# player4771/YOLO-DBL

Measured on AMD Instinct MI355X. Metric: images/sec @640×640 bs=32 (1/2/4/8 GPU) + mAP@0.5 vs CPU ref, higher is better.
Workload: dtype fp16; 1 GPU; YOLO-DBL-n 640x640 bs=32/GPU fp16 forward+decode+NMS (conf .25, iou .7, max_det 300); model=yolov13n_DBL, global_batch=32, imgsz=640, nc=3, parallelism=dp1, streams_per_gpu=2

## Files before the change

### yolo-dbl_amd/csrc/bneck_kernel.hpp

```cpp
#pragma once
#include <algorithm>

#include "common.hpp"
#ifdef YDBL_BNECK_SPARSE
#include "decode_math.hpp"
#endif

namespace ydbl {

struct KSlot {
  int tap, chunk;
  bool live;
};

template <int CH>
__host__ __device__ constexpr KSlot kslot(int m, int g) {
  if constexpr (CH >= 4) {
    return KSlot{m / (CH / 4), (m % (CH / 4)) * 4 + g, true};
  } else if constexpr (CH == 2) {
    const int tap = 2 * m + (g >> 1);
    return KSlot{tap < 9 ? tap : 8, g & 1, tap < 9};
  } else {
    constexpr int taps[3][4] = {{0, 3, 1, 4}, {2, 5, 6, 6}, {7, 7, 8, 8}};
    constexpr bool live[3][4] = {{true, true, true, true}, {true, true, true, false}, {true, false, true, false}};
    return KSlot{taps[m][g], 0, live[m][g]};
  }
}
template <int CH>
constexpr int ksteps() {
  return CH >= 4 ? 9 * CH / 4 : (CH == 2 ? 5 : 3);
}
constexpr int rup16(int v) { return (v + 15) / 16 * 16; }

template <int C, int CMID, int TH, int CIN = C>
struct BneckCfg {
  static constexpr int CM = CMID, CH = CIN / 8, CHM = (CM + 7) / 8;
  static constexpr int NT1 = (CM + 15) / 16, NT2 = C / 16;
  static constexpr bool BD = CM == 8 && CH == 2;
  static constexpr int KS1 = BD ? 9 : ksteps<CH>(), KS2 = ksteps<CHM>();
  static constexpr int TW = 16;
  static constexpr int IP = TW + 4;
  static constexpr int IR = TH + 5;
  static constexpr int NPX = IR * IP;
  static constexpr int PIN = rup16(NPX);
  static constexpr int MR = TH + 2;
  static constexpr int MP = CHM == 1 ? 32 : IP;
  static constexpr int PMID = rup16(MR * MP);
  static constexpr int G1 = (MR * IP + 15) / 16;
  static constexpr int IN_BYTES = CH * PIN * 16, MID_BYTES = CHM * PMID * 16;
  static constexpr int LDS = IN_BYTES + MID_BYTES;
  static constexpr int W1F = NT1 * KS1 * 64, W2F = NT2 * KS2 * 64;
  static constexpr int64_t BYTES = (int64_t)(W1F + W2F) * 16 + (NT1 * 16 + C) * 4;
  static_assert(CH >= 2, "input needs >= 16 channels");
  static_assert((G1 * 16 - 1) + 2 * IP + 2 < NPX, "virtual grid tail must stay inside the window");
};

template <int C, int CMID, int CIN = C>
void bneck_pack(const float* w1, const float* b1, const float* w2, const float* b2, unsigned char* out) {
  using Cfg = BneckCfg<C, CMID, 16, CIN>;
  constexpr int CM = Cfg::CM;
  _Float16* f1 = reinterpret_cast<_Float16*>(out);
  _Float16* f2 = f1 + Cfg::W1F * 8;
  float* fb1 = reinterpret_cast<float*>(f2 + Cfg::W2F * 8);
  float* fb2 = fb1 + Cfg::NT1 * 16;
  if constexpr (Cfg::BD) {
    for (int m = 0; m < Cfg::KS1; ++m)
      for (int lane = 0; lane < 64; ++lane)
        for (int j = 0; j < 8; ++j) {
          const int g = lane >> 4, row = lane & 15;
          const int co = row % 8, ci = (g & 1) * 8 + j;
          f1[(m * 64 + lane) * 8 + j] = (_Float16)((row / 8) == (g >> 1) ? w1[(co * CIN + ci) * 9 + m] : 0.f);
        }
  } else
  for (int t = 0; t < Cfg::NT1; ++t)
    for (int m = 0; m < Cfg::KS1; ++m)
      for (int lane = 0; lane < 64; ++lane)
        for (int j = 0; j < 8; ++j) {
          const KSlot s = kslot<Cfg::CH>(m, lane >> 4);
          const int co = 16 * t + (lane & 15), ci = s.chunk * 8 + j;
          const bool ok = s.live && co < CM;
          f1[((t * Cfg::KS1 + m) * 64 + lane) * 8 + j] = (_Float16)(ok ? w1[(co * CIN + ci) * 9 + s.tap] : 0.f);
        }
  for (int t = 0; t < Cfg::NT2; ++t)
    for (int m = 0; m < Cfg::KS2; ++m)
      for (int lane = 0; lane < 64; ++lane)
        for (int j = 0; j < 8; ++j) {
          const KSlot s = kslot<Cfg::CHM>(m, lane >> 4);
          const int co = 16 * t + (lane & 15), ci = s.chunk * 8 + j;
          const bool ok = s.live && ci < CM;
          f2[((t * Cfg::KS2 + m) * 64 + lane) * 8 + j] = (_Float16)(ok ? w2[(co * CM + ci) * 9 + s.tap] : 0.f);
        }
  for (int i = 0; i < Cfg::NT1 * 16; ++i) fb1[i] = i < CM ? b1[i] : 0.f;
  for (int i = 0; i < C; ++i) fb2[i] = b2[i];
}

template <int CH, int PL, int P>
__device__ __forceinline__ int koff(int m, int g) {
  const KSlot s = kslot<CH>(m, CH >= 4 ? 0 : g);
  return (s.chunk * PL + (s.tap / 3) * P + s.tap % 3) * 16;
}
template <int CH, int PL>
__device__ __forceinline__ int kbase(int g) {
  return CH >= 4 ? g * PL * 16 : 0;
}

#if defined(YDBL_BNECK_STAMPS) && defined(YDBL_BNECK_SPARSE)
#undef YDBL_BNECK_STAMPS
#endif
#ifdef YDBL_BNECK_STAMPS
__device__ unsigned long long g_bn_stamps[8 * 16384];
#define BN_STAMP(k)                                                                                         \
  do {                                                                                                    \
    if (threadIdx.x == 0 && blockIdx.x < 16384) g_bn_stamps[blockIdx.x * 8 + (k)] = __builtin_amdgcn_s_memrealtime(); \
  } while (0)
#else
#define BN_STAMP(k) \
  do {              \
  } while (0)
#endif

#ifdef YDBL_BNECK_SPARSE
struct BoxSink {
  const unsigned char* mask;
  float* cbox;
  const int* cidx;
  const int* ccount;
  int cap, a0, nc, multi;
  float stride;
};
constexpr int BOX_PITCH = 72, BOX_HITS = 512;

#define YDBL_BNECK_KERNEL bneck_sparse_kernel
#define YDBL_BNECK_SINK_ARG , BoxSink sk
#else
#define YDBL_BNECK_KERNEL bneck_kernel
#define YDBL_BNECK_SINK_ARG
#endif

template <int C, int CMID, int TH, bool ADD, bool PW = false, int CIN = C>
__global__ __launch_bounds__(256, 2) void YDBL_BNECK_KERNEL(DView<const _Float16> x, DView<_Float16> y,
                                                            const unsigned char* __restrict__ params, int tiles_x,
                                                            int tiles_y, int ntiles YDBL_BNECK_SINK_ARG) {
  using Cfg = BneckCfg<C, CMID, TH, CIN>;
#ifdef YDBL_BNECK_SPARSE
  static_assert(PW, "the tile mask belongs to the Detect box launch");
#endif
  constexpr int CH = Cfg::CH, CHM = Cfg::CHM, CM = Cfg::CM;
  static_assert(CIN == C || !ADD, "the residual needs c_in == c");
  constexpr bool LATE_A2 = CIN > C;
  constexpr int IP = Cfg::IP, MP = Cfg::MP, PIN = Cfg::PIN, PMID = Cfg::PMID;
  constexpr int NT1 = Cfg::NT1, NT2 = Cfg::NT2, KS1 = Cfg::KS1, KS2 = Cfg::KS2;
  const h8* w1f = reinterpret_cast<const h8*>(params);
  const h8* w2f = w1f + Cfg::W1F;
  const float* b1 = reinterpret_cast<const float*>(w2f + Cfg::W2F);
  const float* b2 = b1 + NT1 * 16;
  __shared__ __align__(16) unsigned char smem[Cfg::LDS];
  unsigned char* s_in = smem;
  unsigned char* s_mid = smem + Cfg::IN_BYTES;

  const int tid = threadIdx.x, lane = tid & 63, wave = wave_id();
  const int g = lane >> 4, r16 = lane & 15;
  BN_STAMP(0);
#ifdef YDBL_BNECK_STAMPS
  if (tid == 0 && blockIdx.x < 16384) {
    unsigned hw, xcc;
    asm volatile("s_getreg_b32 %0, hwreg(HW_REG_HW_ID)" : "=s"(hw));
    asm volatile("s_getreg_b32 %0, hwreg(HW_REG_XCC_ID)" : "=s"(xcc));
    g_bn_stamps[blockIdx.x * 8 + 4] = hw;
    g_bn_stamps[blockIdx.x * 8 + 5] = xcc;
  }
#endif
  const int t = (ntiles & 7) ? (int)blockIdx.x : xcd_remap(blockIdx.x, ntiles);
  const int tx = t % tiles_x, ty = (t / tiles_x) % tiles_y;
  const int img = t / (tiles_x * tiles_y);
  const int oy0 = ty * TH, ox0 = tx * Cfg::TW;
#ifdef YDBL_BNECK_SPARSE
  if (sk.mask[t] == 0) return;
  __shared__ int s_nhit;
  if (tid == 0) s_nhit = 0;
  int ncand = 0, idx0 = -1;
  if (sk.ccount) {
    ncand = min(sk.ccount[img], sk.cap);
    idx0 = sk.cidx[(int64_t)img * sk.cap + min(tid, sk.cap - 1)];
  }
#endif

  static_assert(32 % CH == 0, "staging pattern assumes CH | 32");
  constexpr int PXU = 256 / CH;
  constexpr int IT = (Cfg::NPX + PXU - 1) / PXU;
  const int s_chunk = (tid >> 3) % CH, px0 = ((tid >> 3) / CH) * 8 + (tid & 7);
  h8 xr[IT];
#pragma unroll
  for (int u = 0; u < IT; ++u) {
    const int px = px0 + u * PXU;
    const int r = px / IP, c = px - r * IP;
    const int iy = oy0 - 2 + r, ix = ox0 - 2 + c;
    const bool ok = px < Cfg::NPX && iy >= 0 && iy < x.h && ix >= 0 && ix < x.w;
    const _Float16* src = ok ? x.at(img, iy, ix) + s_chunk * 8 : x.p;
    const h8 v = *reinterpret_cast<const h8*>(src);
    xr[u] = ok ? v : h8{0, 0, 0, 0, 0, 0, 0, 0};
  }
  const int t1 = wave % NT1, t2 = wave % NT2;
  h8 a1[KS1], a2[KS2];
#pragma unroll
  for (int m = 0; m < KS1; ++m) a1[m] = w1f[(t1 * KS1 + m) * 64 + lane];
  if constexpr (!LATE_A2) {
#pragma unroll
    for (int m = 0; m < KS2; ++m) a2[m] = w2f[(t2 * KS2 + m) * 64 + lane];
  }
  unsigned char* s_dst = s_in + (s_chunk * PIN + px0) * 16;
#pragma unroll
  for (int u = 0; u < IT; ++u)
    if (px0 + u * PXU < Cfg::NPX) *reinterpret_cast<h8*>(s_dst + u * PXU * 16) = xr[u];
  float bias1[4], bias2[4];
  const int c1 = Cfg::BD ? 4 * (g & 1) : 16 * t1 + 4 * g;
  const int c2 = 16 * t2 + 4 * g;
#pragma unroll
  for (int q = 0; q < 4; ++q) {
    bias1[q] = b1[c1 + q];
    bias2[q] = b2[c2 + q];
  }
  unsigned char* mid_w = s_mid + ((c1 >> 3) * PMID) * 16 + (c1 & 7) * 2;
  const unsigned char* in_b = s_in + kbase<CH, PIN>(g);
  const bool interior = oy0 >= 1 && ox0 >= 1 && oy0 + TH + 1 <= y.h && ox0 + Cfg::TW + 1 <= y.w;
  __syncthreads();
  BN_STAMP(1);

  auto epi1 = [&](const f32x4& acc, int vr, int vc, int rb) {
    if (vr >= Cfg::MR || c1 >= CM) return;
    bool inside = true;
    if (!interior) {
      const int my = oy0 - 1 + vr, mx = ox0 - 1 + vc;
      inside = my >= 0 && my < y.h && mx >= 0 && mx < y.w;
    }
    h4 o;
#pragma unroll
    for (int q = 0; q < 4; ++q) {
      const float sv = silu_fast(acc[q] + bias1[q]);
      o[q] = f16_rne(inside ? sv : 0.f);
    }
    *reinterpret_cast<h4*>(mid_w + (rb + vc) * 16) = o;
  };
  constexpr int WPT1 = 4 / NT1;
  constexpr int S0 = 2 * WPT1 * 16, H1 = WPT1 * 16;
  int r0, c0, rb0;
  {
    const int v = (wave / NT1) * 16 + r16;
    r0 = v / IP;
    c0 = v - r0 * IP;
    rb0 = r0 * MP;
  }
  for (int gi = wave / NT1; gi < Cfg::G1; gi += 2 * WPT1) {
    const int v0 = gi * 16 + r16;
    const bool two = gi + WPT1 < Cfg::G1;
    const int v1 = two ? v0 + 16 * WPT1 : v0;
    if constexpr (Cfg::BD) {
      const int set = g >> 1;
      const unsigned char* pb = s_in + ((g & 1) * PIN + (set ? v1 : v0)) * 16;
      f32x4 acc = f32x4{0.f, 0.f, 0.f, 0.f};
#pragma unroll
      for (int m = 0; m < KS1; ++m) {
        const h8 bf = *reinterpret_cast<const h8*>(pb + ((m / 3) * IP + m % 3) * 16);
        acc = __builtin_amdgcn_mfma_f32_16x16x32_f16(a1[m], bf, acc, 0, 0, 0);
      }
      const bool w1 = c0 + H1 % IP >= IP;
      const int dr = set ? H1 / IP + (w1 ? 1 : 0) : 0;
      epi1(acc, set && !two ? Cfg::MR : r0 + dr, set ? c0 + H1 % IP - (w1 ? IP : 0) : c0, rb0 + dr * MP);
    } else {
      f32x4 acc0 = f32x4{0.f, 0.f, 0.f, 0.f}, acc1 = acc0;
      const unsigned char* p0 = in_b + v0 * 16;
      const unsigned char* p1 = in_b + v1 * 16;
#pragma unroll
      for (int m = 0; m < KS1; ++m) {
        const int o = koff<CH, PIN, IP>(m, g);
        const h8 bf0 = *reinterpret_cast<const h8*>(p0 + o);
        const h8 bf1 = *reinterpret_cast<const h8*>(p1 + o);
        acc0 = __builtin_amdgcn_mfma_f32_16x16x32_f16(a1[m], bf0, acc0, 0, 0, 0);
        acc1 = __builtin_amdgcn_mfma_f32_16x16x32_f16(a1[m], bf1, acc1, 0, 0, 0);
      }
      epi1(acc0, r0, c0, rb0);
      if (two) {
        const bool w1 = c0 + H1 % IP >= IP;
        const int dr = H1 / IP + (w1 ? 1 : 0);
        epi1(acc1, r0 + dr, c0 + H1 % IP - (w1 ? IP : 0), rb0 + dr * MP);
      }
    }
    const bool w0 = c0 + S0 % IP >= IP;
    const int dr = S0 / IP + (w0 ? 1 : 0);
    c0 += S0 % IP - (w0 ? IP : 0);
    r0 += dr;
    rb0 += dr * MP;
  }

  const unsigned char* res_r = s_in + ((c2 >> 3) * PIN + 2 * IP + 2) * 16 + (c2 & 7) * 2;
  const unsigned char* mid_b = s_mid + kbase<CHM, PMID>(g);
  if constexpr (LATE_A2) {
#pragma unroll
    for (int m = 0; m < KS2; ++m) a2[m] = w2f[(t2 * KS2 + m) * 64 + lane];
  }
  __syncthreads();
  BN_STAMP(2);

  const int64_t lane_px = (int64_t)r16 * y.cs;
  auto epi2 = [&](const f32x4& acc, int j) {
    const int oy = oy0 + j, ox = ox0 + r16;
    if (oy >= y.h || ox >= y.w) return;
    float v[4];
#pragma unroll
    for (int q = 0; q < 4; ++q) v[q] = silu_fast(acc[q] + bias2[q]);
    if constexpr (ADD) {
      const h4 rv = *reinterpret_cast<const h4*>(res_r + (j * IP + r16) * 16);
#pragma unroll
      for (int q = 0; q < 4; ++q) v[q] = float(rv[q]) + v[q];
    }
    if constexpr (PW) {
      h4 o;
#pragma unroll
      for (int q = 0; q < 4; ++q) o[q] = f16_rne(v[q]);
      *reinterpret_cast<h4*>(s_in + ((c2 >> 3) * (TH * 16) + j * 16 + r16) * 16 + (c2 & 7) * 2) = o;
    } else {
      store_f<4>(y.at(img, oy, ox0) + lane_px + c2, v);
    }
  };
  constexpr int WPT2 = 4 / NT2;
  for (int j = wave / NT2; j < TH; j += 2 * WPT2) {
    const bool two = j + WPT2 < TH;
    const int j1 = two ? j + WPT2 : j;
    f32x4 acc0 = f32x4{0.f, 0.f, 0.f, 0.f}, acc1 = acc0;
    const unsigned char* p0 = mid_b + (j * MP + r16) * 16;
    const unsigned char* p1 = mid_b + (j1 * MP + r16) * 16;
#pragma unroll
    for (int m = 0; m < KS2; ++m) {
      const int o = koff<CHM, PMID, MP>(m, g);
      const h8 bf0 = *reinterpret_cast<const h8*>(p0 + o);
      const h8 bf1 = *reinterpret_cast<const h8*>(p1 + o);
      acc0 = __builtin_amdgcn_mfma_f32_16x16x32_f16(a2[m], bf0, acc0, 0, 0, 0);
      acc1 = __builtin_amdgcn_mfma_f32_16x16x32_f16(a2[m], bf1, acc1, 0, 0, 0);
    }
    epi2(acc0, j);
    if (two) epi2(acc1, j1);
  }
  BN_STAMP(3);

  if constexpr (PW) {
    static_assert(ADD == false && C % 32 == 0 && (C / 8) * TH * 16 * 16 <= Cfg::IN_BYTES, "pw stage layout");
    constexpr int NT3 = C / 16, KS3 = C / 32, WPT3 = 4 / NT3;
    const h8* w3f = reinterpret_cast<const h8*>(b2 + C);
    const float* b3 = reinterpret_cast<const float*>(w3f + NT3 * KS3 * 64);
    const int t3 = wave % NT3, c3 = 16 * t3 + 4 * g;
    h8 a3[KS3];
#pragma unroll
    for (int m = 0; m < KS3; ++m) a3[m] = w3f[(t3 * KS3 + m) * 64 + lane];
    float bias3[4];
#pragma unroll
    for (int q = 0; q < 4; ++q) bias3[q] = b3[c3 + q];
    __syncthreads();
#ifdef YDBL_BNECK_SPARSE
    _Float16* s_box = reinterpret_cast<_Float16*>(s_mid);
    int* s_hit = reinterpret_cast<int*>(s_mid + TH * 16 * BOX_PITCH * 2);
    static_assert(C == 64 && TH * 16 * BOX_PITCH * 2 + BOX_HITS * 4 <= Cfg::MID_BYTES, "sink layout");
#endif
    for (int j = wave / NT3; j < TH; j += WPT3) {
      f32x4 acc = f32x4{0.f, 0.f, 0.f, 0.f};
#pragma unroll
      for (int m = 0; m < KS3; ++m) {
        const h8 bf = *reinterpret_cast<const h8*>(s_in + ((m * 4 + g) * (TH * 16) + j * 16 + r16) * 16);
        acc = __builtin_amdgcn_mfma_f32_16x16x32_f16(a3[m], bf, acc, 0, 0, 0);
      }
      const int oy = oy0 + j, ox = ox0 + r16;
      if (oy < y.h && ox < y.w) {
        float v[4];
#pragma unroll
        for (int q = 0; q < 4; ++q) v[q] = acc[q] + bias3[q];
#ifdef YDBL_BNECK_SPARSE
        const h4 o = to_h4_rne(v);
        *reinterpret_cast<h4*>(y.at(img, oy, ox) + c3) = o;
        *reinterpret_cast<h4*>(s_box + (j * 16 + r16) * BOX_PITCH + c3) = o;
#else
        store_f<4>(y.at(img, oy, ox) + c3, v);
#endif
      }
    }
#ifdef YDBL_BNECK_SPARSE
    {
      if (sk.ccount == nullptr) return;
      const int hw = y.h * y.w;
      const int* ci = sk.cidx + (int64_t)img * sk.cap;
      for (int i = tid; i < ncand; i += 256) {
        const int idx = i == tid ? idx0 : ci[i];
        const int loc = (sk.multi ? idx / sk.nc : idx) - sk.a0;
        if (loc < 0 || loc >= hw) continue;
        const int gy = loc / y.w, gx = loc - gy * y.w;
        const int jy = gy - oy0, jx = gx - ox0;
        if (jy < 0 || jy >= TH || jx < 0 || jx >= 16) continue;
        const int h = atomicAdd(&s_nhit, 1);
        if (h < BOX_HITS) s_hit[h] = (i << 7) | (jy * 16 + jx);
      }
      __syncthreads();
      const int nh = min(s_nhit, BOX_HITS);
      const int s = tid & 3;
      for (int h0 = 0; h0 < nh; h0 += 64) {
        const int h = h0 + (tid >> 2);
        const bool live = h < nh;
        const int e = s_hit[live ? h : 0];
        const int px = e & 127;
        const float mine = dfl_side(s_box + px * BOX_PITCH + s * 16);
        const int q0 = lane - s;
        float dist[4];
#pragma unroll
        for (int k = 0; k < 4; ++k) dist[k] = __shfl(mine, q0 + k);
        const f32x4 box = xywh2xyxy(dist2xywh(ox0 + (px & 15), oy0 + (px >> 4), dist, sk.stride));
        if (live && s == 0) *reinterpret_cast<f32x4*>(sk.cbox + ((int64_t)img * sk.cap + (e >> 7)) * 4) = box;
      }
    }
#endif
  }
}

}
```

### yolo-dbl_amd/csrc/sparse_box.hip

```cpp
#define YDBL_DS_DEFER
#define YDBL_BNECK_SPARSE
#include "bneck_kernel.hpp"
#include "dsc_lean.hpp"
#include "dsconv_kernel.hpp"

namespace ydbl {

template <int TH, int CSEG, bool DBUF>
static void ds_defer_go(const ConvArgs<_Float16>& a, const float* dww, const float* dwb, int dw_act, hipStream_t s) {
  const int tiles_x = (int)cdiv(a.Wo, 8), tiles_y = (int)cdiv(a.Ho, TH);
  const int64_t ntiles = (int64_t)a.N * tiles_y * tiles_x;
  dsconv_defer_kernel<_Float16, 3, 1, 1, TH, 8, CSEG, 4, DBUF, true><<<(unsigned)ntiles, 256, 0, s>>>(
      a, dww, dwb, dw_act, tiles_x, tiles_y, 1);
}

bool ds_defer_tile(const ConvArgs<_Float16>& a, const float* dww, const float* dwb, int dw_act, int th, int cseg,
                   bool dbuf, hipStream_t s) {
  if (!a.sk_deferred() || a.Cout != 64) return false;
  if (th == 8 && cseg == 2 && !dbuf) return ds_defer_go<8, 2, false>(a, dww, dwb, dw_act, s), true;
  if (th == 16 && cseg == 4 && !dbuf) return ds_defer_go<16, 4, false>(a, dww, dwb, dw_act, s), true;
  if (th == 8 && cseg == 2 && dbuf) return ds_defer_go<8, 2, true>(a, dww, dwb, dw_act, s), true;
  return false;
}

__global__ __launch_bounds__(256, 1) void dsc_lean_defer_kernel(ConvArgs<_Float16> p, const float* __restrict__ dww,
                                                                 const float* __restrict__ dwb, int dw_act, int tiles_x,
                                                                 int tiles_y, int ntiles) {
  __shared__ __attribute__((aligned(16))) unsigned char smem[LeanLds<64, 64, 3, 1, 8, 8, 256, true>::BYTES];
  lean_tile<64, 64, 3, 1, 8, 8, 256, true, true>(p, dww, dwb, dw_act, xcd_remap(blockIdx.x, ntiles), tiles_x, tiles_y,
                                                 smem);
}

void lean_defer_tile(const ConvArgs<_Float16>& a, const float* dww, const float* dwb, int dw_act, hipStream_t s) {
  const int tiles_x = (int)cdiv(a.Wo, 8), tiles_y = (int)cdiv(a.Ho, 8);
  const int ntiles = a.N * tiles_y * tiles_x;
  dsc_lean_defer_kernel<<<(unsigned)ntiles, 256, 0, s>>>(a, dww, dwb, dw_act, tiles_x, tiles_y, ntiles);
}

__global__ void ds_zero_counts_masks_kernel(int* c, int n, unsigned char* m, int nm) {
  for (int i = threadIdx.x; i < n; i += blockDim.x) c[i] = 0;
  for (int i = threadIdx.x; i < nm; i += blockDim.x) m[i] = 0;
}

void ds_zero_counts_masks(int* counts, int n, unsigned char* masks, int nbytes, hipStream_t s) {
  ds_zero_counts_masks_kernel<<<1, 256, 0, s>>>(counts, n, masks, nbytes);
}

template <int CIN>
static int box_sparse_go(const ydbl_bottleneck_desc* d, hipStream_t s) {
  using Cfg = BneckCfg<64, 64, 8, CIN>;
  const int tiles_x = (int)cdiv(d->y.w, Cfg::TW), tiles_y = (int)cdiv(d->y.h, 8);
  const int64_t nt = (int64_t)tiles_x * tiles_y * d->y.n;
  if (nt > 0x7fffffff) return fail(YDBL_EINVAL, "bottleneck: grid too large");
  const BoxSink sk{d->tile_mask, d->cand_box, d->cand_idx, d->cand_count, d->cand_cap, d->anchor0, d->nc,
                   d->multi_label, d->level_stride};
  bneck_sparse_kernel<64, 64, 8, false, true, CIN><<<(unsigned)nt, 256, 0, s>>>(
      dview<const _Float16>(d->x), dview<_Float16>(d->y), reinterpret_cast<const unsigned char*>(d->params), tiles_x,
      tiles_y, (int)nt, sk);
  return check_launch("ydbl_bottleneck_nhwc");
}

int box_sparse_launch(const ydbl_bottleneck_desc* d, hipStream_t s) {
  return d->x.c == 128 ? box_sparse_go<128>(d, s) : box_sparse_go<64>(d, s);
}

}
```

### yolo-dbl_amd/ydbl/runtime.py

```python

from __future__ import annotations

import ctypes as C
import operator
import os
import time
from dataclasses import dataclass, field

import torch

from . import _lib
from ._lib import View, lib


SWITCHES = ("YDBL_DS2_OFF", "YDBL_DS_LEAN", "YDBL_HG_UNFUSED", "YDBL_HALO_NB", "YDBL_HALO_SMALL", "YDBL_VW", "YDBL_WSK_HALF",
            "YDBL_LSK_FUSE", "YDBL_NMS_FAST", "YDBL_NMS_GROUPS", "YDBL_SPLITK", "YDBL_NO_BNECK", "YDBL_NO_BOX3",
            "YDBL_NO_CLS_TAIL", "YDBL_DWPW", "YDBL_NO_PAIR3", "YDBL_NO_FUSE_PAD", "YDBL_NO_MERGE", "YDBL_NO_STEM2",
            "YDBL_EPI_GENERIC", "YDBL_NO_SPARSE_BOX", "YDBL_NO_HG_PAIR", "YDBL_DW_PAIR_OLD")


def ydbl_env() -> tuple:
    get = os.environ.get
    return tuple(get(k) for k in SWITCHES)


_STRUCT_EPOCH = [0]


def _bump_epoch(*_):
    _STRUCT_EPOCH[0] += 1


for _reg in ("register_module_parameter_registration_hook", "register_module_buffer_registration_hook",
             "register_module_module_registration_hook"):
    getattr(torch.nn.modules.module, _reg)(_bump_epoch)
_VERSION = operator.attrgetter("_version")


def weights_signature(module: torch.nn.Module) -> tuple:
    c = module.__dict__.get("_wsig_cache")
    if c is None or c[0] != _STRUCT_EPOCH[0]:
        ts = [t for t in (*module.parameters(), *module.buffers()) if t.is_floating_point()]
        c = (_STRUCT_EPOCH[0], ts, hash(tuple((id(t), t.data_ptr()) for t in ts)))
        module.__dict__["_wsig_cache"] = c
    return c[2], sum(map(_VERSION, c[1]))


def round_up(x: int, m: int) -> int:
    return (x + m - 1) // m * m


class TV:

    __slots__ = ("base", "off", "n", "h", "w", "c", "cs")

    def __init__(self, base: torch.Tensor, off: int, n: int, h: int, w: int, c: int, cs: int):
        self.base, self.off, self.n, self.h, self.w, self.c, self.cs = base, off, n, h, w, c, cs

    @property
    def dtype(self):
        return self.base.dtype

    @property
    def ptr(self) -> int:
        return self.base.data_ptr() + self.off * self.base.element_size()

    @property
    def shape(self):
        return (self.n, self.h, self.w, self.c)

    def cslice(self, c0: int, c: int) -> "TV":
        assert 0 <= c0 and c0 + c <= self.c, (c0, c, self.c)
        return TV(self.base, self.off + c0, self.n, self.h, self.w, c, self.cs)

    def with_hw(self, h: int, w: int) -> "TV":
        assert h * w == self.h * self.w
        return TV(self.base, self.off, self.n, h, w, self.c, self.cs)

    def struct(self) -> View:
        return View(self.ptr, self.n, self.h, self.w, self.c, self.cs, _lib.dtype_code(self.dtype))

    def torch(self) -> torch.Tensor:
        return torch.as_strided(
            self.base, (self.n, self.h, self.w, self.c), (self.h * self.w * self.cs, self.w * self.cs, self.cs, 1),
            self.off,
        )

    def nchw(self) -> torch.Tensor:
        return self.torch().permute(0, 3, 1, 2)


@dataclass
class Step:
    fn: object
    args: tuple
    what: str
    keep: list = field(default_factory=list)


class Plan:

    def __init__(self, device: torch.device, dtype: torch.dtype):
        self.device = torch.device(device)
        self.dtype = dtype
        self.steps: list[Step] = []
        self.buffers: list[torch.Tensor] = []
        self.bytes_allocated = 0
        self._writers: dict = {}
        self.fp8_candidates: list = []
        self.fp8_layers: list = []

    def alloc(self, n: int, h: int, w: int, c: int, dtype: torch.dtype | None = None, cs: int | None = None) -> TV:
        dtype = dtype or self.dtype
        cs = cs or round_up(c, 8)
        t = torch.empty(n * h * w * cs, dtype=dtype, device=self.device)
        self.buffers.append(t)
        self.bytes_allocated += t.numel() * t.element_size()
        return TV(t, 0, n, h, w, c, cs)

    def scratch(self, nbytes: int, zero: bool = False) -> torch.Tensor:
        t = (torch.zeros if zero else torch.empty)(max(int(nbytes), 16), dtype=torch.uint8, device=self.device)
        self.buffers.append(t)
        self.bytes_allocated += t.numel()
        return t

    def splitk_scratch(self, nbytes: int) -> torch.Tensor:
        cur = getattr(self, "_splitk", None)
        if cur is None or cur.numel() < nbytes:
            cur = self._splitk = self.scratch(nbytes)
        return cur

    def const(self, t: torch.Tensor) -> torch.Tensor:
        t = t.detach().to(self.device).contiguous()
        self.buffers.append(t)
        return t

    def launch(self, name: str, *args, what: str = "", keep=()):
        self.steps.append(Step(getattr(lib, name), args, what or name, list(keep)))

    @staticmethod
    def _vkey(v: TV):
        return (v.base.data_ptr(), v.off, v.n, v.h, v.w, v.c, v.cs)

    def note_writer(self, y: TV, desc) -> None:
        self._writers[self._vkey(y)] = (len(self.steps) - 1, desc)

    def writer_of(self, v: TV):
        return self._writers.get(self._vkey(v))

    def made_before(self, v: TV, step: int) -> bool:
        w = self.writer_of(v)
        return w is not None and w[0] < step

    def fuse_second_output(self, writer, y2: TV, r2: TV, a2: float, b2: float) -> TV | None:
        _, d = writer
        if not hasattr(d, "y2") or d.y2.ptr:
            return None
        y = d.y
        for v in (y2, r2):
            if (v.n, v.h, v.w, v.c) != (y.n, y.h, y.w, y.c) or _lib.dtype_code(v.dtype) != y.dtype or v.cs % 4:
                return None
            if isinstance(d, (_lib.DySampleDesc, _lib.DySample2Desc)):
                vec = 16 // v.base.element_size()
                if v.cs % vec or v.c % vec or v.ptr % 16:
                    return None
        d.y2, d.r2, d.a2, d.b2 = y2.struct(), r2.struct(), float(a2), float(b2)
        self.steps[writer[0]].keep.append((y2, r2))
        return y2

    def check_single_stream(self):
        for st in self.steps:
            if not (isinstance(st.fn, C._CFuncPtr) or getattr(st.fn, "single_stream", False)):
                raise RuntimeError(f"plan step '{st.what}' ({st.fn!r}) is not a single-stream launch: it cannot be "
                                   f"captured as a branch of a split session's graph")

    def run_observed(self, observe, stream: int | None = None):
        s = C.c_void_p(torch.cuda.current_stream(self.device).cuda_stream if stream is None else stream)
        for i, st in enumerate(self.steps):
            observe(i)
            rc = st.fn(*st.args, s)
            if rc:
                _lib.check(rc, st.what)

    def run(self, stream: int | None = None):
        s = C.c_void_p(torch.cuda.current_stream(self.device).cuda_stream if stream is None else stream)
        for st in self.steps:
            rc = st.fn(*st.args, s)
            if rc:
                _lib.check(rc, st.what)

    def run_timed(self):
        stream = torch.cuda.current_stream(self.device)
        s = C.c_void_p(stream.cuda_stream)
        evs = []
        torch.cuda._sleep(int(1e8))
        for st in self.steps:
            a = torch.cuda.Event(enable_timing=True)
            b = torch.cuda.Event(enable_timing=True)
            a.record(stream)
            rc = st.fn(*st.args, s)
            b.record(stream)
            if rc:
                _lib.check(rc, st.what)
            evs.append((st.what, a, b))
        torch.cuda.synchronize(self.device)
        return [(w, a.elapsed_time(b)) for w, a, b in evs]

    def run_graph_timed(self, reps: int = 8, iters: int = 3):
        out = []
        for st in self.steps:
            self.run()
            g = torch.cuda.CUDAGraph()
            with torch.cuda.graph(g):
                s = C.c_void_p(torch.cuda.current_stream(self.device).cuda_stream)
                for _ in range(reps):
                    rc = st.fn(*st.args, s)
                    if rc:
                        _lib.check(rc, st.what)
            g.replay()
            torch.cuda.synchronize(self.device)
            a = torch.cuda.Event(enable_timing=True)
            b = torch.cuda.Event(enable_timing=True)
            best = float("inf")
            for _ in range(iters):
                torch.cuda._sleep(int(2e6))
                a.record()
                g.replay()
                b.record()
                torch.cuda.synchronize(self.device)
                best = min(best, a.elapsed_time(b) / reps)
            out.append((st.what, best))
            del g
        return out


class GraphRunner:

    def __init__(self, plan: Plan, warmup: int = 1, pre: Plan | None = None):
        self.plan = plan
        side = torch.cuda.Stream(plan.device)
        side.wait_stream(torch.cuda.current_stream(plan.device))
        with torch.cuda.stream(side):
            for _ in range(warmup):
                if pre is not None:
                    pre.run(side.cuda_stream)
                plan.run(side.cuda_stream)
        torch.cuda.current_stream(plan.device).wait_stream(side)
        torch.cuda.synchronize(plan.device)
        self.graph = torch.cuda.CUDAGraph()
        with torch.cuda.graph(self.graph):
            if pre is not None:
                pre.run()
            plan.run()
        torch.cuda.synchronize(plan.device)

    def replay(self):
        self.graph.replay()


class BranchGraphRunner:

    def __init__(self, plans, warmup: int = 1, pre: Plan | None = None):
        for p in plans:
            p.check_single_stream()
        dev = plans[0].device
        side = torch.cuda.Stream(dev)
        side.wait_stream(torch.cuda.current_stream(dev))
        with torch.cuda.stream(side):
            for _ in range(warmup):
                if pre is not None:
                    pre.run(side.cuda_stream)
                for p in plans:
                    p.run(side.cuda_stream)
        torch.cuda.current_stream(dev).wait_stream(side)
        torch.cuda.synchronize(dev)
        self.sides = [torch.cuda.Stream(dev) for _ in plans[1:]]
        self.graph = torch.cuda.CUDAGraph()
        with torch.cuda.graph(self.graph):
            cap = torch.cuda.current_stream(dev)
            if pre is not None:
                pre.run()
            for st in self.sides:
                st.wait_stream(cap)
            plans[0].run()
            for p, st in zip(plans[1:], self.sides):
                with torch.cuda.stream(st):
                    p.run(st.cuda_stream)
            for st in self.sides:
                cap.wait_stream(st)
        torch.cuda.synchronize(dev)

    def replay(self):
        self.graph.replay()


def timed(fn, *a, sync_device=None, **k):
    t0 = time.perf_counter()
    r = fn(*a, **k)
    if sync_device is not None:
        torch.cuda.synchronize(sync_device)
    return r, time.perf_counter() - t0
```

Baseline: 19010 images/s.

## Split sparse Detect box tiles into 4-row workgroups and prefetch weights early

The sparse box bottleneck launch now uses 4-row workgroup tiles by default, with 8 rows still selectable through an env switch. Each sub-tile looks up the shared 8-row tile mask, so the grid has more, smaller workgroups for better occupancy and load balance on the sparse launch. In the sub-tile path the third-stage weights, the biases and extra candidate indices are loaded before the first barrier so their latency overlaps input staging. The cost is more halo recompute per output row, a longer candidate scan repeated in each sub-tile, and higher register pressure.

```diff
diff --git a/yolo-dbl_amd/csrc/bneck_kernel.hpp b/yolo-dbl_amd/csrc/bneck_kernel.hpp
--- a/yolo-dbl_amd/csrc/bneck_kernel.hpp
+++ b/yolo-dbl_amd/csrc/bneck_kernel.hpp
@@ -144,6 +144,8 @@
   using Cfg = BneckCfg<C, CMID, TH, CIN>;
 #ifdef YDBL_BNECK_SPARSE
   static_assert(PW, "the tile mask belongs to the Detect box launch");
+  static_assert(TH == 8 || TH == 4 || TH == 2, "a workgroup's rows divide the mask tile's 8");
+  constexpr bool SUB = TH < 8;
 #endif
   constexpr int CH = Cfg::CH, CHM = Cfg::CHM, CM = Cfg::CM;
   static_assert(CIN == C || !ADD, "the residual needs c_in == c");
@@ -175,13 +177,21 @@
   const int img = t / (tiles_x * tiles_y);
   const int oy0 = ty * TH, ox0 = tx * Cfg::TW;
 #ifdef YDBL_BNECK_SPARSE
-  if (sk.mask[t] == 0) return;
+  const int mt = SUB ? (img * ((y.h + 7) >> 3) + (oy0 >> 3)) * tiles_x + tx : t;
+  if (sk.mask[mt] == 0) return;
   __shared__ int s_nhit;
   if (tid == 0) s_nhit = 0;
   int ncand = 0, idx0 = -1;
   if (sk.ccount) {
     ncand = min(sk.ccount[img], sk.cap);
     idx0 = sk.cidx[(int64_t)img * sk.cap + min(tid, sk.cap - 1)];
+  }
+  int idx1 = -1, idx2 = -1;
+  if constexpr (SUB) {
+    if (sk.ccount) {
+      idx1 = sk.cidx[(int64_t)img * sk.cap + min(tid + 256, sk.cap - 1)];
+      idx2 = sk.cidx[(int64_t)img * sk.cap + min(tid + 512, sk.cap - 1)];
+    }
   }
 #endif
 
@@ -208,6 +218,19 @@
 #pragma unroll
     for (int m = 0; m < KS2; ++m) a2[m] = w2f[(t2 * KS2 + m) * 64 + lane];
   }
+#ifdef YDBL_BNECK_SPARSE
+  h8 a3s[SUB ? C / 32 : 1];
+  f32x4 bias1s, bias2s, bias3s;
+  if constexpr (SUB) {
+    const h8* w3s = reinterpret_cast<const h8*>(b2 + C);
+#pragma unroll
+    for (int m = 0; m < C / 32; ++m) a3s[m] = w3s[((wave % (C / 16)) * (C / 32) + m) * 64 + lane];
+    bias1s = *reinterpret_cast<const f32x4*>(b1 + 16 * t1 + 4 * g);
+    bias2s = *reinterpret_cast<const f32x4*>(b2 + 16 * t2 + 4 * g);
+    bias3s = *reinterpret_cast<const f32x4*>(reinterpret_cast<const float*>(w3s + (C / 16) * (C / 32) * 64) +
+                                             16 * (wave % (C / 16)) + 4 * g);
+  }
+#endif
   unsigned char* s_dst = s_in + (s_chunk * PIN + px0) * 16;
 #pragma unroll
   for (int u = 0; u < IT; ++u)
@@ -215,10 +238,21 @@
   float bias1[4], bias2[4];
   const int c1 = Cfg::BD ? 4 * (g & 1) : 16 * t1 + 4 * g;
   const int c2 = 16 * t2 + 4 * g;
-#pragma unroll
-  for (int q = 0; q < 4; ++q) {
-    bias1[q] = b1[c1 + q];
-    bias2[q] = b2[c2 + q];
+#ifdef YDBL_BNECK_SPARSE
+  if constexpr (SUB) {
+#pragma unroll
+    for (int q = 0; q < 4; ++q) {
+      bias1[q] = bias1s[q];
+      bias2[q] = bias2s[q];
+    }
+  } else
+#endif
+  {
+#pragma unroll
+    for (int q = 0; q < 4; ++q) {
+      bias1[q] = b1[c1 + q];
+      bias2[q] = b2[c2 + q];
+    }
   }
   unsigned char* mid_w = s_mid + ((c1 >> 3) * PMID) * 16 + (c1 & 7) * 2;
   const unsigned char* in_b = s_in + kbase<CH, PIN>(g);
@@ -349,11 +383,21 @@
     const float* b3 = reinterpret_cast<const float*>(w3f + NT3 * KS3 * 64);
     const int t3 = wave % NT3, c3 = 16 * t3 + 4 * g;
     h8 a3[KS3];
-#pragma unroll
-    for (int m = 0; m < KS3; ++m) a3[m] = w3f[(t3 * KS3 + m) * 64 + lane];
     float bias3[4];
-#pragma unroll
-    for (int q = 0; q < 4; ++q) bias3[q] = b3[c3 + q];
+#ifdef YDBL_BNECK_SPARSE
+    if constexpr (SUB) {
+#pragma unroll
+      for (int m = 0; m < KS3; ++m) a3[m] = a3s[m];
+#pragma unroll
+      for (int q = 0; q < 4; ++q) bias3[q] = bias3s[q];
+    } else
+#endif
+    {
+#pragma unroll
+      for (int m = 0; m < KS3; ++m) a3[m] = w3f[(t3 * KS3 + m) * 64 + lane];
+#pragma unroll
+      for (int q = 0; q < 4; ++q) bias3[q] = b3[c3 + q];
+    }
     __syncthreads();
 #ifdef YDBL_BNECK_SPARSE
     _Float16* s_box = reinterpret_cast<_Float16*>(s_mid);
@@ -387,7 +431,7 @@
       const int hw = y.h * y.w;
       const int* ci = sk.cidx + (int64_t)img * sk.cap;
       for (int i = tid; i < ncand; i += 256) {
-        const int idx = i == tid ? idx0 : ci[i];
+        const int idx = i == tid ? idx0 : SUB && i == tid + 256 ? idx1 : SUB && i == tid + 512 ? idx2 : ci[i];
         const int loc = (sk.multi ? idx / sk.nc : idx) - sk.a0;
         if (loc < 0 || loc >= hw) continue;
         const int gy = loc / y.w, gx = loc - gy * y.w;
diff --git a/yolo-dbl_amd/csrc/sparse_box.hip b/yolo-dbl_amd/csrc/sparse_box.hip
--- a/yolo-dbl_amd/csrc/sparse_box.hip
+++ b/yolo-dbl_amd/csrc/sparse_box.hip
@@ -46,22 +46,30 @@
   ds_zero_counts_masks_kernel<<<1, 256, 0, s>>>(counts, n, masks, nbytes);
 }
 
-template <int CIN>
+template <int CIN, int TS>
 static int box_sparse_go(const ydbl_bottleneck_desc* d, hipStream_t s) {
-  using Cfg = BneckCfg<64, 64, 8, CIN>;
-  const int tiles_x = (int)cdiv(d->y.w, Cfg::TW), tiles_y = (int)cdiv(d->y.h, 8);
+  using Cfg = BneckCfg<64, 64, TS, CIN>;
+  const int tiles_x = (int)cdiv(d->y.w, Cfg::TW), tiles_y = (int)cdiv(d->y.h, TS);
   const int64_t nt = (int64_t)tiles_x * tiles_y * d->y.n;
   if (nt > 0x7fffffff) return fail(YDBL_EINVAL, "bottleneck: grid too large");
   const BoxSink sk{d->tile_mask, d->cand_box, d->cand_idx, d->cand_count, d->cand_cap, d->anchor0, d->nc,
                    d->multi_label, d->level_stride};
-  bneck_sparse_kernel<64, 64, 8, false, true, CIN><<<(unsigned)nt, 256, 0, s>>>(
+  bneck_sparse_kernel<64, 64, TS, false, true, CIN><<<(unsigned)nt, 256, 0, s>>>(
       dview<const _Float16>(d->x), dview<_Float16>(d->y), reinterpret_cast<const unsigned char*>(d->params), tiles_x,
       tiles_y, (int)nt, sk);
   return check_launch("ydbl_bottleneck_nhwc");
 }
 
 int box_sparse_launch(const ydbl_bottleneck_desc* d, hipStream_t s) {
-  return d->x.c == 128 ? box_sparse_go<128>(d, s) : box_sparse_go<64>(d, s);
+  const bool deep = d->x.c == 128;
+  int ts = 4;
+  const char* e = getenv("YDBL_BOX_SUBTILE");
+  if (e && e[0]) {
+    if ((e[0] != '8' && e[0] != '4') || e[1]) return fail(YDBL_EINVAL, "YDBL_BOX_SUBTILE must be 8 or 4");
+    ts = e[0] - '0';
+  }
+  if (ts == 4) return deep ? box_sparse_go<128, 4>(d, s) : box_sparse_go<64, 4>(d, s);
+  return deep ? box_sparse_go<128, 8>(d, s) : box_sparse_go<64, 8>(d, s);
 }
 
 }
diff --git a/yolo-dbl_amd/ydbl/runtime.py b/yolo-dbl_amd/ydbl/runtime.py
--- a/yolo-dbl_amd/ydbl/runtime.py
+++ b/yolo-dbl_amd/ydbl/runtime.py
@@ -16,7 +16,8 @@
 SWITCHES = ("YDBL_DS2_OFF", "YDBL_DS_LEAN", "YDBL_HG_UNFUSED", "YDBL_HALO_NB", "YDBL_HALO_SMALL", "YDBL_VW", "YDBL_WSK_HALF",
             "YDBL_LSK_FUSE", "YDBL_NMS_FAST", "YDBL_NMS_GROUPS", "YDBL_SPLITK", "YDBL_NO_BNECK", "YDBL_NO_BOX3",
             "YDBL_NO_CLS_TAIL", "YDBL_DWPW", "YDBL_NO_PAIR3", "YDBL_NO_FUSE_PAD", "YDBL_NO_MERGE", "YDBL_NO_STEM2",
-            "YDBL_EPI_GENERIC", "YDBL_NO_SPARSE_BOX", "YDBL_NO_HG_PAIR", "YDBL_DW_PAIR_OLD")
+            "YDBL_EPI_GENERIC", "YDBL_NO_SPARSE_BOX", "YDBL_NO_HG_PAIR", "YDBL_DW_PAIR_OLD",
+            "YDBL_BOX_SUBTILE")
 
 
 def ydbl_env() -> tuple:
```

Result: no change. 19090 images/s, median of 6 (+0.4%).
